# EdwardSmith1884/GEOMetrics

Hardware: AMD Instinct MI355X
Metric: meshes/sec (sample+Chamfer+tri_dist+0N-GCN fwd+bwd), 2562 verts/3000 pts (higher is better)
Workload: dtype f32; 1 GPU; BASELINE config 5 shard: 8 independent 2562-vert/5120-face meshes per GPU, full loss (face sampling 3000 pts + Chamfer NN vs 3000 GT pts + tri_distance 3000x5120 + point-to-surface) on top of a 3-layer 0N-GCN 963-192-192-192, fwd+bwd, single process (no collective), Adam step; meshes_per_gpu=8, global_batch=8, parallelism=dp1, launch=hipgraph, gemm_selection=tunableop file

## Files before the change

### geometrics_amd/build.py

```python
import glob
import os
import subprocess
import sys

HERE = os.path.dirname(os.path.abspath(__file__))
CSRC = os.path.join(HERE, "csrc")
INCLUDE = os.path.join(os.path.dirname(HERE), "include")
LIBDIR = os.path.join(HERE, "lib")
LIB = os.path.join(LIBDIR, "libgeom_hip.so")
STAMP = os.path.join(LIBDIR, "libgeom_hip.digest")
SHIM = os.path.join(LIBDIR, "geom_torch_shim.so")
SHIM_SRC = os.path.join(CSRC, "torch_shim.cpp")

HIPCC_FLAGS = ["--offload-arch=gfx950", "-O3", "-std=c++17", "-ffp-contract=off", "-fPIC",
               "-fno-gpu-rdc", "-fno-slp-vectorize", "-Wall", "-Wno-unused-function"]


EXTRA_FLAGS = {"dense_gemm.hip": ["-mllvm", "-amdgpu-mfma-vgpr-form=1"],
               "zn_stack.hip": ["-mllvm", "-amdgpu-mfma-vgpr-form=1"],
               "deform_block.hip": ["-mllvm", "-amdgpu-mfma-vgpr-form=1"],
               "encoder_stack.hip": ["-mllvm", "-amdgpu-mfma-vgpr-form=1"]}


def sources():
    return sorted(glob.glob(os.path.join(CSRC, "*.hip")))


def source_digest():
    import hashlib
    h = hashlib.sha256()
    for path in sorted(sources() + glob.glob(os.path.join(CSRC, "*.h")) + glob.glob(os.path.join(INCLUDE, "*.h"))):
        h.update(os.path.basename(path).encode())
        with open(path, "rb") as f:
            h.update(f.read())
    return h.hexdigest()


def _stale():
    if not os.path.exists(LIB):
        return True
    if built_digest() not in (None, source_digest()):
        return True
    t = os.path.getmtime(LIB)
    deps = sources() + glob.glob(os.path.join(CSRC, "*.h")) + glob.glob(os.path.join(INCLUDE, "*.h"))
    return any(os.path.getmtime(d) > t for d in deps)


def build_shim(force=False, verbose=False):
    if not force and os.path.exists(SHIM) and os.path.getmtime(SHIM) >= max(os.path.getmtime(SHIM_SRC), os.path.getmtime(LIB)):
        return SHIM
    import sysconfig
    import torch
    from torch.utils import cpp_extension as ce
    tlib = ce.library_paths()[0]
    cmd = ["g++", "-O2", "-std=c++17", "-fPIC", "-shared", "-w", "-D__HIP_PLATFORM_AMD__=1", "-DUSE_ROCM=1",
           "-DTORCH_EXTENSION_NAME=geom_torch_shim", "-D_GLIBCXX_USE_CXX11_ABI=%d" % int(torch._C._GLIBCXX_USE_CXX11_ABI),
           "-I", INCLUDE, "-I", sysconfig.get_paths()["include"], "-I", "/opt/rocm/include"]
    for inc in ce.include_paths():
        cmd += ["-I", inc]
    cmd += [SHIM_SRC, "-o", SHIM, "-L", LIBDIR, "-lgeom_hip", "-L", tlib, "-ltorch", "-ltorch_cpu", "-ltorch_hip", "-lc10",
            "-lc10_hip", "-ltorch_python", "-Wl,-rpath,$ORIGIN", "-Wl,-rpath," + tlib]
    if verbose:
        print(" ".join(cmd))
    subprocess.check_call(cmd)
    return SHIM


def build(force=False, verbose=False):
    lib = build_lib(force, verbose)
    build_shim(force, verbose)
    return lib


def build_lib(force=False, verbose=False):
    if not force and not _stale():
        return LIB
    hipcc = os.environ.get("HIPCC", "/opt/rocm/bin/hipcc")
    os.makedirs(LIBDIR, exist_ok=True)
    objs = []
    procs = []
    for src in sources():
        obj = os.path.join(LIBDIR, os.path.basename(src)[:-4] + ".o")
        objs.append(obj)
        cmd = [hipcc] + HIPCC_FLAGS + EXTRA_FLAGS.get(os.path.basename(src), []) + ["-I", INCLUDE, "-I", CSRC, "-c", src, "-o", obj]
        if verbose:
            print(" ".join(cmd))
        procs.append((src, subprocess.Popen(cmd, stdout=subprocess.PIPE, stderr=subprocess.STDOUT)))
    for src, p in procs:
        out, _ = p.communicate()
        if p.returncode != 0:
            raise RuntimeError("hipcc failed on %s:\n%s" % (src, out.decode(errors="replace")))
        if verbose and out:
            print(out.decode(errors="replace"))
    cmd = [hipcc, "--offload-arch=gfx950", "-shared", "-fPIC", "-fno-gpu-rdc"] + objs + ["-o", LIB]
    subprocess.check_call(cmd)
    with open(STAMP, "w") as f:
        f.write(source_digest() + "\n")
    return LIB


def built_digest():
    try:
        with open(STAMP) as f:
            return f.read().strip() or None
    except OSError:
        return None


if __name__ == "__main__":
    print(build(force="--force" in sys.argv, verbose=True))
```

### geometrics_amd/dense.py

```python
import ctypes

import torch

from . import _lib


def supported(cin, c, rows=1):
    return 0 < c <= 192 and c % 16 == 0 and cin > 0 and rows * max(cin, c) < 2 ** 30


def plan(rows, cin, c):
    ok = supported(cin, c, rows)
    pair = ok and cin <= 192 and cin % 4 == 0 and rows >= 512
    ok = ok and c % 48 == 0
    pair = pair and ok
    return {"fwd": "lib", "dx": "mfma" if pair else "lib", "dw": "mfma" if ok and rows >= 512 else "lib", "pair": pair}


def forward(x, w, out=None):
    rows, cin = x.shape
    c = w.shape[1]
    out = torch.empty(rows, c, dtype=torch.float32, device=x.device) if out is None else out
    with torch.cuda.device(x.device):
        _lib.call("geom_dense_fwd_f32", rows, cin, c, x.data_ptr(), w.data_ptr(), 0, None, out.data_ptr(), None, None)
    return out


def forward_split(x, w, bias, ksplit, out, sup, mask):
    rows, cin = x.shape
    c = w.shape[1]
    with torch.cuda.device(x.device):
        _lib.call("geom_dense_fwd_f32", rows, cin, c, x.data_ptr(), w.data_ptr(), ksplit, _lib.ptr(bias), out.data_ptr(),
                  sup.data_ptr(), _lib.ptr(mask))


def backward_input(g, w, out=None):
    rows, c = g.shape
    cin = w.shape[0]
    out = torch.empty(rows, cin, dtype=torch.float32, device=g.device) if out is None else out
    with torch.cuda.device(g.device):
        _lib.call("geom_dense_bwd_input_f32", rows, cin, c, g.data_ptr(), w.data_ptr(), out.data_ptr())
    return out


def weight_workspace(rows, cin, c, device):
    n = int(_lib.lib().geom_dense_bwd_weight_workspace_floats(rows, cin, c))
    return torch.empty(n, dtype=torch.float32, device=device)


launch_probe = None


def backward_weight_partials(x, g, workspace, want_colsum=False):
    rows, cin = x.shape
    c = g.shape[1]
    probe = launch_probe
    with torch.cuda.device(x.device):
        if probe is not None:
            start, end = torch.cuda.Event(enable_timing=True), torch.cuda.Event(enable_timing=True)
            start.record()
        _lib.call("geom_dense_bwd_weight_f32", rows, cin, c, x.data_ptr(), g.data_ptr(), workspace.data_ptr(),
                  1 if want_colsum else 0)
        if probe is not None:
            end.record()
            probe.append((rows, cin, c, start, end))


def backward_pair(x, g, w, grad_x, workspace, want_colsum=False):
    rows, cin = x.shape
    c = g.shape[1]
    with torch.cuda.device(x.device):
        _lib.call("geom_dense_bwd_f32", rows, cin, c, x.data_ptr(), g.data_ptr(), w.data_ptr(), grad_x.data_ptr(),
                  workspace.data_ptr(), 1 if want_colsum else 0)


def reduce(jobs, stream=None):
    n = len(jobs)
    if n == 0:
        return
    if n > _lib.DENSE_MAX_LAYERS:
        for i in range(0, n, _lib.DENSE_MAX_LAYERS):
            reduce(jobs[i:i + _lib.DENSE_MAX_LAYERS], stream)
        return
    ints = lambda k: (ctypes.c_int * n)(*[j[k] for j in jobs])
    ptrs = lambda k: (ctypes.c_void_p * n)(*[None if j[k] is None else j[k].data_ptr() for j in jobs])
    dev = jobs[0][3].device
    with torch.cuda.device(dev):
        _lib.check(_lib.status("geom_dense_reduce_f32", n, ints(0), ints(1), ints(2), ptrs(3), ptrs(4), ptrs(5), stream=stream),
                   "geom_dense_reduce_f32")


def backward_weight(x, g, want_bias=False):
    rows, cin = x.shape
    c = g.shape[1]
    ws = weight_workspace(rows, cin, c, x.device)
    backward_weight_partials(x, g, ws, want_bias)
    gw = torch.empty(cin, c, dtype=torch.float32, device=x.device)
    gb = torch.empty(c, dtype=torch.float32, device=x.device) if want_bias else None
    reduce([(rows, cin, c, ws, gw, gb)])
    return gw, gb


def any_supported(rows, cin, c):
    return rows >= 256 and cin > 0 and c > 0 and rows * max(cin, c) * 4 < 2 ** 31 - 1


def _row_major(t):
    return t.dim() == 2 and t.stride(1) == 1 and t.stride(0) >= t.shape[1]


def gemm(a, b, trans_a=False, trans_b=False, out=None, workspace=None):
    if not (_row_major(a) and _row_major(b)):
        raise ValueError("gemm operands must be 2-D with contiguous rows")
    for name, t in (("a", a), ("b", b), ("out", out), ("workspace", workspace)):
        if t is None:
            continue
        if not t.is_cuda or t.dtype != torch.float32:
            raise ValueError("gemm: %s must be a float32 tensor on a HIP device (got %s on %s)" % (name, t.dtype, t.device))
        if t.device != a.device:
            raise ValueError("gemm: %s is on %s, a on %s" % (name, t.device, a.device))
    k, m = (a.shape if trans_a else a.shape[::-1])
    n, kb = (b.shape if trans_b else b.shape[::-1])
    if k != kb:
        raise ValueError("gemm: summed extents differ (%d vs %d)" % (k, kb))
    if out is None:
        out = torch.empty(m, n, dtype=torch.float32, device=a.device)
    elif not _row_major(out) or tuple(out.shape) != (m, n):
        raise ValueError("gemm: out must be [%d, %d] with contiguous rows" % (m, n))
    need = int(_lib.lib().geom_gemm_workspace_floats(m, n, k))
    if need and (workspace is None or workspace.numel() < need):
        workspace = torch.empty(need, dtype=torch.float32, device=a.device)
    with torch.cuda.device(a.device):
        _lib.call("geom_gemm_f32", m, n, k, a.data_ptr(), a.stride(0), 1 if trans_a else 0, b.data_ptr(), b.stride(0),
                  0 if trans_b else 1, out.data_ptr(), out.stride(0), _lib.ptr(workspace) if need else None, need)
    return out


def split_bf16_planes(w):
    if not (w.is_cuda and w.dtype == torch.float32 and w.dim() == 2 and w.is_contiguous()):
        raise ValueError("split_bf16_planes: a contiguous 2-D float32 tensor on a HIP device")
    k, n = w.shape
    kpad = int(_lib.lib().geom_split_bf16_kpad(k))
    planes = torch.empty(3, n, kpad, dtype=torch.int16, device=w.device)
    with torch.cuda.device(w.device):
        _lib.call("geom_split_bf16_planes_f32", k, n, w.data_ptr(), planes.data_ptr())
    return planes


def gemm_split_bf16(a, planes, terms=6, out=None):
    if not (a.is_cuda and a.dtype == torch.float32 and a.dim() == 2 and a.is_contiguous()):
        raise ValueError("gemm_split_bf16: a contiguous 2-D float32 tensor on a HIP device")
    m, k = a.shape
    n = planes.shape[1]
    if planes.shape[2] != int(_lib.lib().geom_split_bf16_kpad(k)):
        raise ValueError("gemm_split_bf16: the planes belong to another k")
    out = torch.empty(m, n, dtype=torch.float32, device=a.device) if out is None else out
    with torch.cuda.device(a.device):
        _lib.call("geom_gemm_split_bf16_f32", m, k, n, a.data_ptr(), planes.data_ptr(), out.data_ptr(), int(terms))
    return out
```

### geometrics_amd/products.py

```python
import os
import threading
from collections import namedtuple

import torch

from . import backward_pass as _pass
from . import dense as _dense_kernels
from . import gemm_tuning


class _Slabs:
    def __init__(self, slots):
        self.open = {}
        self.slots = max(2, int(slots))

    def take(self, kind, shape, device, descending=False):
        shape = tuple(shape)
        key = (kind, shape, device, descending)
        slots = self.slots
        cur = self.open.get(key)
        if cur is None or cur[1] == slots:
            cur = self.open[key] = [torch.empty((slots,) + shape, dtype=torch.float32, device=device), 0]
        index = slots - 1 - cur[1] if descending else cur[1]
        cur[1] += 1
        return cur[0][index]


_active = threading.local()


def current_slabs():
    return getattr(_active, "slabs", None)


class weight_gradient_batching:

    def __init__(self, depth=4):
        self.depth = depth

    def __enter__(self):
        self.outer = current_slabs()
        _active.slabs = _Slabs(self.depth) if torch.is_grad_enabled() else None
        return self

    def __exit__(self, *exc):
        _active.slabs = self.outer
        return False


def _new_like(t, kind, arena, descending=False):
    if arena is None:
        return torch.empty_like(t)
    return arena.take(kind, t.shape, t.device, descending)


def _regular_run(tensors):
    first = tensors[0]
    if len(tensors) == 1:
        return first, 0
    base = first.untyped_storage().data_ptr()
    if any(t.untyped_storage().data_ptr() != base or t.stride() != first.stride() for t in tensors):
        return None
    step = tensors[1].storage_offset() - first.storage_offset()
    if step <= 0 or any(tensors[i + 1].storage_offset() - tensors[i].storage_offset() != step for i in range(len(tensors) - 1)):
        return None
    return first, step


def _launch_weight_products(jobs):
    i = 0
    while i < len(jobs):
        first = jobs[i]
        j = i + 1
        while (j < len(jobs) and jobs[j].x.shape == first.x.shape and jobs[j].g.shape == first.g.shape
               and jobs[j].stream == first.stream):
            j += 1
        group = jobs[i:j]
        with torch.cuda.stream(first.stream), torch.no_grad():
            runs = [_regular_run([getattr(job, name) for job in group]) for name in ("x", "g", "out")] if len(group) > 1 else None
            if runs and all(runs):
                xb, gb, ob = (torch.as_strided(run[0], (len(group),) + tuple(t.shape), (run[1],) + tuple(t.stride()))
                              for run, t in zip(runs, (first.x, first.g, first.out)))
                torch.bmm(xb.transpose(1, 2), gb, out=ob)
            else:
                for job in group:
                    dw = route(job.x.shape[0], job.x.shape[1], job.g.shape[1], True, True, True, True, False, use_any_shape_products).dw
                    _weight_product(dw, job.x, job.g, out=job.out)
        i = j


use_any_shape_products = True

own_dense_products = None


def _own_products_preferred():
    if own_dense_products is not None:
        return bool(own_dense_products)
    env = os.environ.get("GEOM_OWN_PRODUCTS")
    if env is not None:
        return env not in ("", "0")
    return gemm_tuning.status == "library default (tuning file rejected)"


Route = namedtuple("Route", "forward dx dw node")


def route(rows, cin, c, w_requires_grad, w_contiguous, x_contiguous, batched, own, any_allowed):
    plan = _dense_kernels.plan(rows, cin, c)
    split = plan["dw"] == "mfma"
    any_shape = any_allowed and not split and _dense_kernels.any_supported(rows, cin, c)
    lib_or_own = "own" if (own and w_contiguous and c % 16 == 0 and rows >= 512 and _dense_kernels.supported(cin, c, rows)) else "lib"
    forward = "any" if any_shape and w_contiguous else lib_or_own
    if batched:
        return Route(forward, lib_or_own, "any" if any_shape else "lib", True)
    if split and w_requires_grad:
        if x_contiguous and w_contiguous:
            return Route(forward, "pair" if plan["pair"] else lib_or_own, "split", True)
        return Route(forward, lib_or_own, "lib", lib_or_own == "own")
    if forward == "any":
        return Route("any", "any", "any", True)
    return Route(forward, lib_or_own, "lib", lib_or_own == "own")


def _input_gradient(kind, g, w2, out=None):
    if kind == "any":
        return _dense_kernels.gemm(g, w2, trans_b=True, out=out)
    if kind == "own":
        return _dense_kernels.backward_input(g, w2, out=out)
    return torch.matmul(g, w2.t()) if out is None else torch.mm(g, w2.t(), out=out)


def _weight_product(kind, x2, g2, out=None):
    if kind == "any" and x2.stride(1) == 1 and g2.stride(1) == 1 and (out is None or (out.dim() == 2 and out.stride(1) == 1)):
        return _dense_kernels.gemm(x2, g2, trans_a=True, out=out)
    return torch.mm(x2.t(), g2) if out is None else torch.mm(x2.t(), g2, out=out)


def product_gradients(x, g, w, w_ref, route, need_x, need_w, arena=None, dx=None, leaf=None):
    w2 = w.reshape(w.shape[-2:])
    cin, c = w2.shape
    x2, g2 = x.reshape(-1, cin), g.view(-1, c)
    rows = g2.shape[0]
    need_x = need_x and dx is None
    if route.dw == "split" and need_w:
        ws = _dense_kernels.weight_workspace(rows, cin, c, x.device)
        if need_x and route.dx == "pair":
            dx = torch.empty_like(x)
            _dense_kernels.backward_pair(x2, g2, w2, dx.view(rows, cin), ws)
        else:
            if need_x and leaf is not None and _pass.may_postpone_input_gradient(leaf):
                late = torch.empty(rows, cin, dtype=x.dtype, device=x.device)
                _pass.postpone_input_gradient(lambda: _input_gradient(route.dx, g2, w2, out=late), late, leaf)
            elif need_x:
                dx = _input_gradient(route.dx, g2, w2).view(x.shape)
            _dense_kernels.backward_weight_partials(x2, g2, ws)
        return dx, _pass.weight_gradient(w_ref, w, rows, cin, c, ws)
    if need_x:
        dx = _input_gradient(route.dx, g if arena is not None and route.dx == "lib" else g2, w2).view(x.shape)
    grad_w = None
    if need_w:
        param = w_ref() if arena is not None else None
        if param is not None and x2.is_contiguous() and _pass.may_defer(param, opted_in=True):
            grad_w = arena.take("dW", w.shape, w.device, descending=True)
            _pass.postpone_weight_product(x2, g2, grad_w, w_ref, _launch_weight_products)
        else:
            grad_w = _weight_product(route.dw, x2, g2).view(w.shape)
    return dx, grad_w


class _Product(torch.autograd.Function):

    @staticmethod
    def forward(ctx, x, w, route, arena):
        ctx.route, ctx.arena = route, arena
        ctx.w_ref = _pass.parameter_ref(w, ctx, ctx.needs_input_grad[1])
        x, out = _forward(route.forward, x, w.reshape(w.shape[-2:]))
        ctx.save_for_backward(x, w)
        return out

    @staticmethod
    def backward(ctx, grad):
        x, w = ctx.saved_tensors
        dx, dw = product_gradients(x, grad.contiguous(), w, ctx.w_ref, ctx.route, ctx.needs_input_grad[0], ctx.needs_input_grad[1],
                                   ctx.arena, leaf=x)
        return dx, dw, None, None


def _forward(kind, x, w2):
    if kind == "lib":
        return x, torch.matmul(x, w2)
    x2 = x.reshape(-1, x.shape[-1])
    if not x2.is_contiguous():
        x2 = x2.contiguous()
        x = x2.view(x.shape)
    out = _dense_kernels.gemm(x2, w2) if kind == "any" else _dense_kernels.forward(x2, w2)
    return x, out.view(x.shape[:-1] + (w2.shape[1],))


def _dense(x, w):
    if not (x.is_cuda and x.dtype == torch.float32 and w.dtype == torch.float32
            and (w.dim() == 2 or (w.dim() == 3 and w.shape[0] == 1)) and x.shape[-1] == w.shape[-2]):
        return torch.matmul(x, w.squeeze(0) if w.dim() == 3 else w)
    differentiable = torch.is_grad_enabled() and (x.requires_grad or w.requires_grad)
    arena = current_slabs() if differentiable else None
    cin = x.shape[-1]
    r = route(x.numel() // max(cin, 1), cin, w.shape[-1], w.requires_grad, w.is_contiguous(),
              x.is_contiguous() or x.reshape(-1, cin).is_contiguous(), arena is not None, _own_products_preferred(),
              use_any_shape_products)
    if differentiable and r.node:
        return _Product.apply(x, w, r, arena)
    return _forward(r.forward, x, w.reshape(w.shape[-2:]))[1]
```

### include/geom_hip.h

```cpp
#ifndef GEOM_HIP_H
#define GEOM_HIP_H

#include <stddef.h>
#include <stdint.h>

#ifdef __cplusplus
extern "C" {
#endif

#define GEOM_ABI_VERSION 16

#define GEOM_EINVAL   (-1)
#define GEOM_ETOOBIG  (-2)
#define GEOM_EUNSUPPORTED (-3)

#define GEOM_FLAG_REF_TAIL_TRUNC 1u
#define GEOM_FLAG_FIX_REGION6    2u
#define GEOM_FLAG_TRI_BRUTE_FORCE 4u
#define GEOM_FLAG_NN_FMA 8u

#define GEOM_FLAG_TRI_WS_READY 16u

int geom_abi_version(void);
const char *geom_strerror(int code);

int geom_chamfer_nn_f32(int b, int n, const float *xyz, int m, const float *xyz2,
                        float *result, int *result_i, float *result2, int *result2_i,
                        unsigned flags, void *stream);

int64_t geom_chamfer_nn_culled_workspace_floats(int b, int n, int m);
int geom_chamfer_nn_culled_f32(int b, int n, const float *xyz, int m, const float *xyz2, const int *order1, const int *order2,
                               float *result, int *result_i, float *result2, int *result2_i, unsigned flags, float *workspace,
                               void *stream);

int geom_tri_distance_f32(int b, int n, const float *xyz, int m,
                          const float *tri1, const float *tri2, const float *tri3,
                          float *dist, int *point, int *index, unsigned flags, void *stream);

int geom_tri_distance_indexed_f32(int b, int n, const float *xyz, int nv, const float *verts,
                                  int nf, const int64_t *faces,
                                  float *dist, int *point, int *index, unsigned flags, void *stream);

size_t geom_tri_distance_workspace_bytes(int b, int n, int m);
int geom_tri_distance_ws_f32(int b, int n, const float *xyz, int m,
                             const float *tri1, const float *tri2, const float *tri3, const int *order,
                             float *dist, int *point, int *index, unsigned flags,
                             void *workspace, size_t workspace_bytes, void *stream);
int geom_tri_distance_indexed_ws_f32(int b, int n, const float *xyz, int nv, const float *verts,
                                     int nf, const int64_t *faces, const int *order,
                                     float *dist, int *point, int *index, unsigned flags,
                                     void *workspace, size_t workspace_bytes, void *stream);

int geom_tri_surface_fwd_f32(int b, int n, const float *xyz, int nv, const float *verts, int nf,
                             const int64_t *faces, const int *order, float *dist, int *point, int *index,
                             float *sqdist, float *closest, float *weights, unsigned flags, void *workspace,
                             size_t workspace_bytes, void *stream);

int geom_face_areas_f32(int b, int nv, const float *verts, int nf, const int64_t *faces,
                        float *areas, void *stream);
int geom_draw_samples_f32(int b, int nv, const float *verts, int nf, const int64_t *faces, int num,
                          const float *uniforms, int64_t *choices, float *u, float *v, void *stream);
int geom_draw_samples_rng_f32(int b, int nv, const float *verts, int nf, const int64_t *faces, int num,
                              uint64_t *rng_state, int64_t *choices, float *u, float *v, float *points,
                              void *stream);
int geom_sample_faces_fwd_f32(int b, int nv, const float *verts, int nf, const int64_t *faces,
                              int num, const int64_t *choices, const float *u, const float *v,
                              float *points, void *stream);
int geom_sample_faces_bwd_f32(int b, int nv, int nf, const int64_t *faces,
                              int num, const int64_t *choices, const float *u, const float *v,
                              const float *grad_points, float *grad_verts, void *stream);

int geom_chamfer_grad_f32(int b, int n, const float *src, int m, const float *dst,
                          const int *idx, const float *coef_dev, float coef_host,
                          float *grad_src, int accumulate, float *grad_dst, void *stream);

int geom_p2tri_loss_fwd_f32(int b, int n, const float *xyz, int nv, const float *verts,
                            int nf, const int64_t *faces, const int *option, const int *index,
                            float *sqdist, float *closest, float *weights, void *stream);
int geom_p2tri_loss_bwd_f32(int b, int n, const float *xyz, int nv, int nf, const int64_t *faces,
                            const int *index, const float *closest, const float *weights,
                            const float *coef_dev, float coef_host, float *grad_verts, void *stream);

int geom_sum_f32(int64_t n, const float *x, float scale, float *out, void *stream);

int geom_sample_chamfer_bwd_f32(int b, int nv, int nf, const int64_t *faces, int num,
                                const int64_t *choices, const float *u, const float *v,
                                const float *points, int n_other, const float *other,
                                const int *idx, int via_nn, const float *coef_dev, float coef_host,
                                float *grad_verts, void *stream);
int geom_surface_loss_bwd_f32(int b, int nv, int nf, const int64_t *faces, int num, const int64_t *choices,
                              const float *u, const float *v, const float *points, int n_gt, const float *gt,
                              const int *idx_g, const int *index, const float *closest, const float *weights,
                              const float *coef_dev, float coef_sample, float coef_tri, float *grad_verts,
                              void *stream);

int geom_zn_gcn_aggregate_fwd_f32(int b, int nv, int c, int k, const int *rowptr, const int *col,
                                  const float *val, const float *support, const float *bias,
                                  int act, float *out, void *stream);
int64_t geom_zn_gcn_bwd_scratch_floats(int b, int nv, int c);
int64_t geom_zn_gcn_bwd_partial_rows(int b, int nv, int c, int k, int ell_w);
#define GEOM_COLSUM_MAX_JOBS 32
int geom_colsum_batch_f32(int count, const float *const *partials, const int *rows, const int *cols,
                          float *const *outs, void *stream);
int geom_zn_gcn_aggregate_bwd_f32(int b, int nv, int c, int k, const int *rowptrT, const int *colT,
                                  const float *valT, const float *grad_out, const float *out,
                                  int act, float *grad_support, float *grad_bias, float *scratch,
                                  void *stream);

int64_t geom_zn_gcn_relu_mask_words(int b, int nv, int c, int k);
int geom_zn_gcn_aggregate_ell_fwd_f32(int b, int nv, int c, int k, int w, const int *ell_col,
                                      const float *ell_val, const int *over_ptr, const int *over_col,
                                      const float *over_val, const float *support, const float *bias,
                                      int act, float *out, uint16_t *relu_mask, void *stream);
int geom_zn_gcn_aggregate_ell_bwd_f32(int b, int nv, int c, int k, int w, const int *ell_colT,
                                      const float *ell_valT, const int *over_ptrT, const int *over_colT,
                                      const float *over_valT, const float *grad_out, const float *out,
                                      const uint16_t *relu_mask, int act, float *grad_support,
                                      float *grad_bias, float *scratch, void *stream);

#define GEOM_DENSE_MAX_LAYERS 8
#define GEOM_DENSE_MAX_REDUCE_JOBS 32
int geom_dense_fwd_f32(int rows, int cin, int c, const float *x, const float *w, int ksplit, const float *bias,
                       float *out, float *sup, uint16_t *mask, void *stream);
int geom_dense_bwd_input_f32(int rows, int cin, int c, const float *g, const float *w, float *grad_x, void *stream);
int64_t geom_dense_bwd_weight_workspace_floats(int rows, int cin, int c);
int geom_dense_bwd_weight_f32(int rows, int cin, int c, const float *x, const float *g, float *workspace,
                              int want_colsum, void *stream);
int geom_dense_bwd_f32(int rows, int cin, int c, const float *x, const float *g, const float *w, float *grad_x,
                       float *workspace, int want_colsum, void *stream);
int geom_dense_reduce2_f32(int count, const int *rows, const int *cin, const int *c, const float *const *workspaces,
                           float *const *grad_w, float *const *grad_bias, int ncs, const float *const *cs_partials,
                           const int *cs_rows, const int *cs_cols, float *const *cs_outs, void *stream);
int geom_dense_reduce_adam_f32(int count, const int *rows, const int *cin, const int *c, const float *const *workspaces,
                               float *const *grad_w, float *const *w_p, float *const *w_m, float *const *w_v, int ncs,
                               const float *const *cs_partials, const int *cs_rows, const int *cs_cols, float *const *cs_outs,
                               float *const *b_p, float *const *b_m, float *const *b_v, float lr, float beta1, float beta2,
                               float eps, float *state, void *stream);
int geom_dense_reduce_f32(int count, const int *rows, const int *cin, const int *c, const float *const *workspaces,
                          float *const *grad_w, float *const *grad_bias, void *stream);

int geom_zn_gcn_aggregate_ell_head_fwd_f32(int b, int nv, int c, int k, int w, const int *ell_col,
                                           const float *ell_val, const int *over_ptr, const int *over_col,
                                           const float *over_val, const float *support, const float *bias,
                                           int act, float *out, uint16_t *relu_mask, const float *base,
                                           float scale, float *pos, void *stream);
int geom_zn_gcn_aggregate_ell_head_bwd_f32(int b, int nv, int c, int k, int w, const int *ell_colT,
                                           const float *ell_valT, const int *over_ptrT, const int *over_colT,
                                           const float *over_valT, const float *grad_pos, float scale,
                                           const uint16_t *relu_mask, int act, float *grad_support,
                                           float *grad_bias, float *scratch, void *stream);

int64_t geom_zn_layer_partial_rows(int b, int nv);
int geom_zn_layer_fwd_f32(int b, int nv, int c, int k, int ell_w, const int *ell_col, const float *ell_val,
                          const float *s_prev, const float *bias_prev, int act, const float *w, int n_out,
                          float *x_out, uint16_t *relu_mask, float *s_out, float *wt_out, void *stream);
int geom_zn_layer_bwd_f32(int b, int nv, int c, int k, int ell_w, const int *ell_col_t, const float *ell_val_t,
                          const float *grad_out, const float *out, const uint16_t *relu_mask, int act,
                          const float *grad_pos, float head_scale, const float *wt, int n_in, float *g_out,
                          float *grad_in, float *colsum_partial, void *stream);

typedef struct geom_deform_fwd {
    int b, nv, c, k, ell_w;
    const float *s_in, *bias;
    const int *ell_col; const float *ell_val;
    const int *tail_col; const float *tail_val;
    const float *bn_w, *bn_b;
    float *run_mean, *run_var;
    int training; float momentum, eps;
    int relu;
    const float *res; int res_ld; float scale;
    float *z_out, *x_out, *save_mean, *save_invstd;
    const float *w_next; float *s_out;
    const float *w_head; float *s_head;
    int vpx;
} geom_deform_fwd;
typedef struct geom_deform_bwd {
    int b, nv, c, k, ell_w;
    const float *dz_up;
    const int *ell_col_t; const float *ell_val_t;
    const int *tail_col_t; const float *tail_val_t;
    float *ds_up; const float *wt_up;
    const float *g, *g2;
    int g_ld, g2_ld;
    const float *z, *bn_w, *bn_b, *save_mean, *save_invstd;
    int relu, has_res; float scale;
    float *grad_res, *dz, *grad_bn_w, *grad_bn_b, *colsum;
    const float *ds_head, *w_head, *x_top; float *dw_head;
    int vpx;
} geom_deform_bwd;
#define GEOM_DEFORM_CHAIN_MAX 13
int geom_deform_chain_fits(int nv);
int geom_deform_chain_fwd_f32(int count, const geom_deform_fwd *layers, int *done, void *stream);
int geom_deform_chain_bwd_f32(int count, const geom_deform_bwd *layers, int *done, float *ds_first, void *stream);
int geom_deform_pack_weights_zero_f32(int count, const float *const *w, float *fwd, float *bwd, int *zero, int zero_words,
                                      void *stream);
typedef struct geom_deform_infer {
    int b, nv, c, k, ell_w;
    const float *s_in, *bias;
    const int *ell_col; const float *ell_val;
    const int *tail_col; const float *tail_val;
    const float *bn_w, *bn_b;
    const float *run_mean, *run_var;
    float eps;
    int relu;
    const float *res; int res_ld; float scale;
    float *x_out;
    const float *w_next; float *s_out;
    const float *w_head; float *s_head;
} geom_deform_infer;
int geom_deform_infer_fwd_f32(const geom_deform_infer *args, void *stream);
int geom_split_bf16_kpad(int k);
int geom_split_bf16_planes_f32(int k, int n, const float *w, uint16_t *planes, void *stream);
int geom_gemm_split_bf16_f32(int m, int k, int n, const float *a, const uint16_t *planes, float *c, int terms, void *stream);

int64_t geom_stage_regularisers_blocks(int b, int nv, int nf);
int geom_stage_regularisers_fwd_f32(int b, int nv, const float *prev, int prev_batched, const float *cur, int nf,
                                    const int64_t *faces, const int *rowptr, const int *col, const float *inv_deg,
                                    float c_lap, float c_move, float c_edge, float *lapd, float *partial, void *stream);
int geom_stage_regularisers_bwd_f32(int b, int nv, const float *prev, int prev_batched, const float *cur, int nf,
                                    const int64_t *faces, const int *rowptr, const int *col, const float *inv_deg,
                                    const int *vf_ptr, const int *vf_item, float c_lap, float c_move, float c_edge,
                                    const float *lapd, const float *gout, float *grad_prev, float *grad_cur, void *stream);

#define GEOM_SUM_MAX_TENSORS 8
int geom_sum_tensors_f32(int count, const float *const *tensors, int64_t n, float *out, void *stream);
int geom_sum_tensors_rows_f32(int count, const float *const *tensors, const int64_t *lds, int64_t rows, int width, float *out,
                              void *stream);

int geom_camera_info_f32(int b, const float *param, float *cam_mat, float *cam_pos, void *stream);

#define GEOM_DEFORM_MAX_PACK 16
#define GEOM_DEFORM_TAIL 32
int geom_deform_pack_weights_f32(int count, const float *const *w, float *fwd, float *bwd, void *stream);
int geom_deform_layer_fwd_f32(const geom_deform_fwd *args, void *stream);
int geom_deform_layer_bwd_f32(const geom_deform_bwd *args, void *stream);
#define GEOM_DEFORM_WIDE_MAX_B 64
int geom_deform_layer_wide_fwd_f32(const geom_deform_fwd *args, void *stream);
int geom_deform_layer_wide_bwd_f32(const geom_deform_bwd *args, void *stream);

int64_t geom_gemm_workspace_floats(int m, int n, int k);
int geom_gemm_f32(int m, int n, int k, const float *a, int64_t lda, int a_km, const float *b, int64_t ldb, int b_kn,
                  float *c, int64_t ldc, float *workspace, int64_t workspace_floats, void *stream);

int geom_vertex_head_fwd_f32(int64_t rows, int c, const float *base, const float *feat, float scale,
                             float *pos, void *stream);
int geom_vertex_head_bwd_f32(int64_t rows, int c, const float *grad_pos, float scale, float *grad_feat,
                             void *stream);

int geom_laplacian_f32(int b, int nv, const int *rowptr, const int *col, const float *inv_deg,
                       const float *x, int transpose, float *out, void *stream);
int geom_edge_sqlen_fwd_f32(int b, int nv, const float *verts, int nf, const int64_t *faces,
                            float *per_face, void *stream);
int geom_edge_sqlen_bwd_f32(int b, int nv, const float *verts, int nf, const int64_t *faces,
                            const float *coef_dev, float coef_host, float *grad_verts, void *stream);

int geom_vertex_bn_fwd_f32(int b, int nv, int c, const float *x, const float *weight, const float *bias,
                           float *running_mean, float *running_var, int training, float momentum, float eps,
                           int relu, const float *residual, int residual_ld, float scale,
                           float *out, float *save_mean, float *save_invstd, void *stream);
int geom_vertex_bn_bwd_f32(int b, int nv, int c, const float *x, const float *grad_out, const float *weight,
                           const float *bias, const float *save_mean, const float *save_invstd, int relu,
                           int has_residual, float scale, float *grad_x, float *grad_residual,
                           float *grad_weight, float *grad_bias, const float *grad_out2, void *stream);

size_t geom_pool_features_bwd_workspace_bytes(int b, int nv, int levels, const int *dims);
#define GEOM_POOL_MAX_LEVELS 8
int geom_pool_features_fwd_ld_f32(int b, int nv, const float *verts, const float *cam_mat, const float *cam_pos, int levels,
                                  const float *const *blocks, const int *channels, const int *dims, float *out, int64_t out_ld,
                                  void *stream);
int geom_pool_features_fwd_fronts_f32(int b, int nv, const float *verts, const float *cam_mat, const float *cam_pos, int levels,
                                      const float *const *blocks, const int *channels, const int *dims, float *out,
                                      int64_t out_ld, int n_fronts, const float *const *fronts, const int *widths,
                                      const int *cols, float *buf, void *stream);
int geom_pool_features_bwd_ld_f32(int b, int nv, const float *verts, const float *cam_mat, const float *cam_pos, int levels,
                                  const float *const *blocks, const int *channels, const int *dims, const float *grad_out,
                                  int64_t grad_ld, float *const *grad_blocks, float *grad_verts, void *workspace,
                                  size_t workspace_bytes, void *stream);

typedef struct geom_surface_cull {
    const int *gt_order;
    const float *gt_index;
    float *sample_index;
    const int *faces_in_order;
} geom_surface_cull;
int64_t geom_nn_cull_index_floats(int b, int n);
int geom_nn_cull_index_f32(int b, int n, const float *xyz, const int *order, float *index, void *stream);

int geom_surface_prepare_f32(int b, int nv, const float *verts, int nf, const int64_t *faces, int num,
                             uint64_t *rng_state, int64_t *choices, float *u, float *v, float *points, int n_gt,
                             const int *tri_order, unsigned flags, void *workspace, size_t workspace_bytes,
                             int *prepared, const geom_surface_cull *cull, void *stream);

size_t geom_surface_tail_counters_offset(int b, int n_gt, int nf);
typedef struct geom_surface_tail {
    const int64_t *choices;
    float scale_sample, scale_other;
    int want_order;
    float *loss;
    int finalized;
} geom_surface_tail;
int geom_surface_scan_f32(int b, int n_gt, const float *gt, int num, const float *points, float *sq_gt, int *idx_p,
                          float *sq_pred, int *idx_g, int nv, const float *verts, int nf, const int64_t *faces,
                          const int *tri_order, float *tri_dist, int *option, int *index, float *sq, float *closest,
                          float *weights, const float *u, const float *v, float coef_sample, float coef_other,
                          int *order_scratch, unsigned flags, void *workspace, size_t workspace_bytes,
                          int *records_written, const geom_surface_cull *cull, geom_surface_tail *tail, void *stream);

int64_t geom_surface_order_words(int b, int nf, int num, int n_gt);
int geom_surface_finalize_f32(int b, int nf, int num, const int64_t *choices, const float *u, const float *v,
                              const float *points, int n_gt, const float *gt, const int *idx_g, const int *idx_p,
                              const int *index, const float *closest, const float *weights, const float *sq_sample,
                              const float *sq_other, float scale_sample, float scale_other, float coef_sample,
                              float coef_other, int want_order, int records_ready, int *order, float *loss,
                              void *stream);
int geom_surface_gather_f32(int b, int nv, int nf, const int *vf_ptr, const int *vf_item, int num, int n_gt,
                            int has_other, const int *order, const float *grad, float *grad_verts, void *stream);
int geom_surface_finalize_w_f32(int b, int nf, int num, const int64_t *choices, const float *u, const float *v,
                                const float *points, int n_gt, const float *gt, const int *idx_g, const int *idx_p,
                                const int *index, const float *closest, const float *weights, const float *sq_sample,
                                const float *sq_other, float scale_sample, float scale_other, float coef_sample,
                                float coef_other, int want_order, int records_ready, int *order, float *loss,
                                const float *mesh_weight, void *stream);
int geom_surface_gather_w_f32(int b, int nv, int nf, const int *vf_ptr, const int *vf_item, int num, int n_gt,
                              int has_other, const int *order, const float *grad, const float *mesh_weight,
                              float *grad_verts, void *stream);

int64_t geom_segment_max_workspace_bytes(int nseg, int c, int64_t max_len);
int geom_segment_max_fwd_f32(int nseg, const int64_t *offsets, int64_t max_len, int c, const float *x,
                             float *out, int *arg, void *workspace, int64_t workspace_bytes, void *stream);
int geom_segment_max_bwd_f32(int nseg, const int64_t *offsets, int64_t total_rows, int c,
                             const float *grad_out, const int *arg, float *grad_x, void *stream);

int geom_encoder_layer_fwd_f32(int b, int nv, int c, int k, int n, const int *rowptr, const int *col, const float *val,
                               const float *s, int64_t lds, const float *bias, int act, const float *w, int64_t ldw,
                               float *out, int64_t ldo, float *x_out, int64_t ldx, void *stream);
int geom_encoder_layer_bwd_f32(int b, int nv, int c, int k, int n, const int *rowptrT, const int *colT, const float *valT,
                               const float *g, int64_t ldg, const float *x_saved, int64_t ldx, int act, const float *w,
                               int64_t ldw, float *out, int64_t ldo, float *t_out, int64_t ldt, void *stream);
int geom_latent_l1_fwd_f32(int b, int l, const float *pred, const float *target, const float *on, float weight, float *loss,
                           void *stream);
int geom_latent_l1_bwd_f32(int b, int l, const float *pred, const float *target, const float *on, float weight,
                           const float *grad_loss, float *grad_pred, void *stream);

#define GEOM_ADAM_MAX_TENSORS 64
#define GEOM_ADAM_STATE_WORDS 2112
int geom_adam_step_f32(int count, float *const *params, const float *const *grads, float *const *exp_avg,
                       float *const *exp_avg_sq, const int64_t *sizes, float lr, float beta1, float beta2,
                       float eps, float grad_scale, float *state, int advance, void *stream);
int64_t geom_adam_table_bytes(int count, int64_t total_blocks);
int geom_adam_table_step_f32(int count, const void *table, int64_t total_blocks, const float *lr, float beta1, float beta2,
                             float eps, float grad_scale, float *state, int advance, void *stream);

#ifdef __cplusplus
}
#endif
#endif
```

Baseline: 17780 meshes/s.

## Add split-bf16 MFMA kernel for wide-input dense backward dx

Adds a HIP kernel that computes the input gradient of a dense layer with 192 outputs and wide input. It splits fp32 operands into three bf16 planes and accumulates six bf16 MFMA products so the result stays near fp32 accuracy. The products fallback routes large wide-input dx products (at least 16384 rows) to this kernel instead of torch.matmul. It also adds a per-call weight plane-conversion launch and rounding behaviour that differs from the fp32 GEMM.

After: 18620 meshes/s, median of 6. +4.7%, better.

```diff
diff --git a/geometrics_amd/build.py b/geometrics_amd/build.py
--- a/geometrics_amd/build.py
+++ b/geometrics_amd/build.py
@@ -19,7 +19,8 @@
 EXTRA_FLAGS = {"dense_gemm.hip": ["-mllvm", "-amdgpu-mfma-vgpr-form=1"],
                "zn_stack.hip": ["-mllvm", "-amdgpu-mfma-vgpr-form=1"],
                "deform_block.hip": ["-mllvm", "-amdgpu-mfma-vgpr-form=1"],
-               "encoder_stack.hip": ["-mllvm", "-amdgpu-mfma-vgpr-form=1"]}
+               "encoder_stack.hip": ["-mllvm", "-amdgpu-mfma-vgpr-form=1"],
+               "dense_dx_split_bf16.hip": ["-mllvm", "-amdgpu-mfma-vgpr-form=1"]}
 
 
 def sources():
diff --git a/geometrics_amd/csrc/dense_dx_split_bf16.hip b/geometrics_amd/csrc/dense_dx_split_bf16.hip
--- /dev/null
+++ b/geometrics_amd/csrc/dense_dx_split_bf16.hip
@@ -0,0 +1,296 @@
+#include "geom_common.h"
+#include <type_traits>
+
+namespace {
+
+typedef float f32x4 __attribute__((ext_vector_type(4)));
+typedef __bf16 bf16x8 __attribute__((ext_vector_type(8)));
+typedef unsigned u32x4 __attribute__((ext_vector_type(4)));
+
+constexpr int DX_THREADS = 256;
+constexpr int DX_K = 192;
+constexpr int DX_KB = DX_K / 32;
+constexpr int DX_NT = 2;
+constexpr int DX_MAX_RB = 6;
+constexpr int DX_ROW_BYTES = DX_K * 2;
+constexpr int DX_PLANE = DX_MAX_RB * 16 * DX_ROW_BYTES;
+constexpr int DX_LDS = 3 * DX_PLANE;
+
+__device__ __forceinline__ unsigned bf16_bits_of(float x) { return (unsigned)__builtin_bit_cast(unsigned short, (__bf16)x); }
+__device__ __forceinline__ float bf16_value_of(unsigned bits) { return __uint_as_float(bits << 16); }
+__device__ __forceinline__ void split3(float a, unsigned &b0, unsigned &b1, unsigned &b2)
+{
+    b0 = bf16_bits_of(a);
+    const float r1 = a - bf16_value_of(b0);
+    b1 = bf16_bits_of(r1);
+    const float r2 = r1 - bf16_value_of(b1);
+    b2 = bf16_bits_of(r2);
+}
+
+__host__ __device__ __forceinline__ size_t dx_frag_index(int group, int kb, int t, int plane, int lane)
+{
+    return ((((size_t)group * DX_KB + kb) * DX_NT + t) * 3 + plane) * 64 + lane;
+}
+
+__global__ __launch_bounds__(256) void dx_planes_kernel(int cin, int cinpad, const float *w, uint4 *planes)
+{
+    const int i = blockIdx.x * 256 + threadIdx.x;
+    if (i >= cinpad * (DX_K / 8)) return;
+    const int col = i / (DX_K / 8), k8 = i - col * (DX_K / 8);
+    unsigned e[8][3];
+#pragma unroll
+    for (int j = 0; j < 8; ++j) e[j][0] = e[j][1] = e[j][2] = 0;
+    if (col < cin) {
+        const float4 lo = *reinterpret_cast<const float4 *>(w + (size_t)col * DX_K + 8 * k8);
+        const float4 hi = *reinterpret_cast<const float4 *>(w + (size_t)col * DX_K + 8 * k8 + 4);
+        const float v[8] = {lo.x, lo.y, lo.z, lo.w, hi.x, hi.y, hi.z, hi.w};
+#pragma unroll
+        for (int j = 0; j < 8; ++j) split3(v[j], e[j][0], e[j][1], e[j][2]);
+    }
+    const int tile = col >> 4;
+#pragma unroll
+    for (int pl = 0; pl < 3; ++pl)
+        planes[dx_frag_index(tile / DX_NT, k8 >> 2, tile % DX_NT, pl, 16 * (k8 & 3) + (col & 15))] =
+            make_uint4(e[0][pl] | (e[1][pl] << 16), e[2][pl] | (e[3][pl] << 16), e[4][pl] | (e[5][pl] << 16), e[6][pl] | (e[7][pl] << 16));
+}
+
+constexpr unsigned DX_NOWHERE = 0x80000000u;
+__device__ __forceinline__ __amdgpu_buffer_rsrc_t dx_rsrc(const void *ptr, int64_t bytes)
+{
+    return __builtin_amdgcn_make_buffer_rsrc(const_cast<void *>(ptr), 0, (int)bytes, 0x00020000);
+}
+
+struct DxArgs {
+    const float *g;
+    const void *wp;
+    float *dx;
+    int rows, cin, cinpad, ldx, spread;
+};
+
+__device__ __forceinline__ int lds_chunk(int r, int q) { return r * DX_ROW_BYTES + ((q ^ ((r >> 1) & 7)) << 4); }
+
+__device__ __forceinline__ void dx_terms(const bf16x8 (&a)[3], const bf16x8 (&b)[DX_NT][3], f32x4 (&hi)[DX_NT], f32x4 (&lo)[DX_NT])
+{
+#pragma unroll
+    for (int t = 0; t < DX_NT; ++t) hi[t] = __builtin_amdgcn_mfma_f32_16x16x32_bf16(a[0], b[t][0], hi[t], 0, 0, 0);
+#pragma unroll
+    for (int t = 0; t < DX_NT; ++t) lo[t] = __builtin_amdgcn_mfma_f32_16x16x32_bf16(a[0], b[t][1], lo[t], 0, 0, 0);
+#pragma unroll
+    for (int t = 0; t < DX_NT; ++t) lo[t] = __builtin_amdgcn_mfma_f32_16x16x32_bf16(a[1], b[t][0], lo[t], 0, 0, 0);
+#pragma unroll
+    for (int t = 0; t < DX_NT; ++t) lo[t] = __builtin_amdgcn_mfma_f32_16x16x32_bf16(a[1], b[t][1], lo[t], 0, 0, 0);
+#pragma unroll
+    for (int t = 0; t < DX_NT; ++t) lo[t] = __builtin_amdgcn_mfma_f32_16x16x32_bf16(a[0], b[t][2], lo[t], 0, 0, 0);
+#pragma unroll
+    for (int t = 0; t < DX_NT; ++t) lo[t] = __builtin_amdgcn_mfma_f32_16x16x32_bf16(a[2], b[t][0], lo[t], 0, 0, 0);
+}
+
+__device__ __forceinline__ void dx_store(const DxArgs &p, __amdgpu_buffer_rsrc_t r_dx, int rb, int grp, int lane, const f32x4 (&hi)[DX_NT],
+                                         const f32x4 (&lo)[DX_NT])
+{
+    const int row = rb * 16 + 4 * (lane >> 4), col = grp * (16 * DX_NT) + (lane & 15);
+#pragma unroll
+    for (int e = 0; e < 4; ++e)
+#pragma unroll
+        for (int t = 0; t < DX_NT; ++t) {
+            const unsigned off = row + e < p.rows && col + 16 * t < p.cin ? (unsigned)(((row + e) * p.ldx + col + 16 * t) * 4) : DX_NOWHERE;
+#ifdef DX_PROBE_NO_STORE
+            if (p.ldx < 0)
+#endif
+            __builtin_amdgcn_raw_buffer_store_b32(__float_as_uint(hi[t][e] + lo[t][e]), r_dx, off, 0, 0);
+        }
+}
+
+template <int N>
+__device__ __forceinline__ void dx_sweep(const DxArgs &p, const unsigned char *lds, int wave, int lane, int rb0)
+{
+    const int lr = lane & 15, lg = lane >> 4;
+    const int ngroups = p.cinpad / (16 * DX_NT);
+    bf16x8 bf[2][DX_KB][DX_NT][3];
+    bf16x8 af[2][3];
+    const __amdgpu_buffer_rsrc_t r_w = dx_rsrc(p.wp, (int64_t)3 * p.cinpad * DX_K * 2);
+    const __amdgpu_buffer_rsrc_t r_dx = dx_rsrc(p.dx, ((int64_t)(p.rows - 1) * p.ldx + p.cin) * 4);
+    auto a_frags = [&](int set, int rbi, int kb) {
+#pragma unroll
+        for (int pl = 0; pl < 3; ++pl)
+            af[set][pl] = *reinterpret_cast<const bf16x8 *>(lds + pl * DX_PLANE + lds_chunk(rbi * 16 + lr, 4 * kb + lg));
+    };
+    auto b_frags = [&](int set, int grp, int kb) {
+        const unsigned base = grp < ngroups ? (unsigned)(dx_frag_index(grp, 0, 0, 0, lane) * 16) : DX_NOWHERE;
+#pragma unroll
+        for (int t = 0; t < DX_NT; ++t)
+#pragma unroll
+            for (int pl = 0; pl < 3; ++pl)
+                bf[set][kb][t][pl] = __builtin_bit_cast(bf16x8, __builtin_amdgcn_raw_buffer_load_b128(r_w, base + (unsigned)(dx_frag_index(0, kb, t, pl, 0) * 16), 0, 0));
+    };
+    auto group = [&](auto set_c, int grp, int next) {
+        constexpr int S = decltype(set_c)::value;
+#pragma unroll
+        for (int rbi = 0; rbi < N; ++rbi) {
+            f32x4 hi[DX_NT], lo[DX_NT];
+#pragma unroll
+            for (int t = 0; t < DX_NT; ++t) hi[t] = lo[t] = (f32x4){0.f, 0.f, 0.f, 0.f};
+#ifndef DX_PROBE_NO_REFILL
+#pragma unroll
+            for (int kb = rbi * DX_KB / N; kb < (rbi + 1) * DX_KB / N; ++kb) b_frags(S ^ 1, next, kb);
+#endif
+#pragma unroll
+            for (int kb = 0; kb < DX_KB; ++kb) {
+                const int s = kb & 1;
+#ifndef DX_PROBE_NO_LDS
+                if (kb + 1 < DX_KB) a_frags(s ^ 1, rbi, kb + 1);
+                else a_frags(0, rbi + 1 < N ? rbi + 1 : 0, 0);
+                __builtin_amdgcn_sched_barrier(0);
+#endif
+                dx_terms(af[s], bf[S][kb], hi, lo);
+            }
+            dx_store(p, r_dx, rb0 + rbi, grp, lane, hi, lo);
+        }
+    };
+
+    if (wave >= ngroups) return;
+#pragma unroll
+    for (int kb = 0; kb < DX_KB; ++kb) b_frags(0, wave, kb);
+#ifdef DX_PROBE_NO_REFILL
+#pragma unroll
+    for (int kb = 0; kb < DX_KB; ++kb) b_frags(1, wave, kb);
+#endif
+    a_frags(0, 0, 0);
+    for (int grp = wave; grp < ngroups; grp += 8) {
+        group(std::integral_constant<int, 0>(), grp, grp + 4);
+        if (grp + 4 < ngroups) group(std::integral_constant<int, 1>(), grp + 4, grp + 8);
+    }
+}
+
+__device__ __forceinline__ void dx_stray(const DxArgs &p, const unsigned char *lds, int lane, int lds_rb, int rb, int grp)
+{
+    const int lr = lane & 15, lg = lane >> 4;
+    const __amdgpu_buffer_rsrc_t r_w = dx_rsrc(p.wp, (int64_t)3 * p.cinpad * DX_K * 2);
+    const __amdgpu_buffer_rsrc_t r_dx = dx_rsrc(p.dx, ((int64_t)(p.rows - 1) * p.ldx + p.cin) * 4);
+    bf16x8 b[DX_KB][DX_NT][3];
+#pragma unroll
+    for (int kb = 0; kb < DX_KB; ++kb)
+#pragma unroll
+        for (int t = 0; t < DX_NT; ++t)
+#pragma unroll
+            for (int pl = 0; pl < 3; ++pl)
+                b[kb][t][pl] = __builtin_bit_cast(bf16x8, __builtin_amdgcn_raw_buffer_load_b128(r_w, (unsigned)(dx_frag_index(grp, kb, t, pl, lane) * 16), 0, 0));
+    f32x4 hi[DX_NT], lo[DX_NT];
+#pragma unroll
+    for (int t = 0; t < DX_NT; ++t) hi[t] = lo[t] = (f32x4){0.f, 0.f, 0.f, 0.f};
+#pragma unroll
+    for (int kb = 0; kb < DX_KB; ++kb) {
+        bf16x8 a[3];
+#pragma unroll
+        for (int pl = 0; pl < 3; ++pl) a[pl] = *reinterpret_cast<const bf16x8 *>(lds + pl * DX_PLANE + lds_chunk(lds_rb * 16 + lr, 4 * kb + lg));
+        dx_terms(a, b[kb], hi, lo);
+    }
+    dx_store(p, r_dx, rb, grp, lane, hi, lo);
+}
+
+__global__ __launch_bounds__(DX_THREADS, 1) void dx_split_kernel(DxArgs p)
+{
+    extern __shared__ __attribute__((aligned(16))) unsigned char lds[];
+    const int tid = threadIdx.x, wave = tid >> 6, lane = tid & 63;
+    const int nrb = (p.rows + 15) >> 4;
+    int rb0 = (int)((int64_t)blockIdx.x * nrb / gridDim.x), n = (int)((int64_t)(blockIdx.x + 1) * nrb / gridDim.x) - rb0;
+    int stray_rb = -1, stray_grp = 0;
+    if (p.spread) {
+        const int ngroups = p.cinpad / (16 * DX_NT), share = nrb / (int)gridDim.x;
+        rb0 = blockIdx.x * share, n = share;
+        if ((int)blockIdx.x < (nrb - share * (int)gridDim.x) * ngroups) stray_rb = share * gridDim.x + blockIdx.x / ngroups, stray_grp = blockIdx.x % ngroups;
+    }
+
+#ifndef DX_PROBE_NO_PROLOGUE
+    {
+        const __amdgpu_buffer_rsrc_t r_g = dx_rsrc(p.g, (int64_t)p.rows * DX_K * 4);
+        u32x4 v[3 * DX_MAX_RB];
+#pragma unroll
+        for (int i = 0; i < 3 * DX_MAX_RB; ++i) {
+            const int q = tid + DX_THREADS * i, r = q / (DX_K / 4);
+            const int row = r < 16 * n ? rb0 * 16 + r : stray_rb * 16 + r - 16 * n;
+            const unsigned off = r < 16 * n || (stray_rb >= 0 && r < 16 * n + 16) ? (unsigned)((row * DX_K + 4 * (q - r * (DX_K / 4))) * 4) : DX_NOWHERE;
+            v[i] = __builtin_amdgcn_raw_buffer_load_b128(r_g, off, 0, 0);
+        }
+#pragma unroll
+        for (int i = 0; i < 3 * DX_MAX_RB; ++i) {
+            const int q = tid + DX_THREADS * i, r = q / (DX_K / 4), c4 = q - r * (DX_K / 4);
+            unsigned e[4][3];
+            split3(__uint_as_float(v[i].x), e[0][0], e[0][1], e[0][2]);
+            split3(__uint_as_float(v[i].y), e[1][0], e[1][1], e[1][2]);
+            split3(__uint_as_float(v[i].z), e[2][0], e[2][1], e[2][2]);
+            split3(__uint_as_float(v[i].w), e[3][0], e[3][1], e[3][2]);
+            unsigned char *dst = lds + lds_chunk(r, c4 >> 1) + 8 * (c4 & 1);
+#pragma unroll
+            for (int pl = 0; pl < 3; ++pl)
+                *reinterpret_cast<uint2 *>(dst + pl * DX_PLANE) = make_uint2(e[0][pl] | (e[1][pl] << 16), e[2][pl] | (e[3][pl] << 16));
+        }
+    }
+#endif
+    __syncthreads();
+    switch (n) {
+    case 1: dx_sweep<1>(p, lds, wave, lane, rb0); break;
+    case 2: dx_sweep<2>(p, lds, wave, lane, rb0); break;
+    case 3: dx_sweep<3>(p, lds, wave, lane, rb0); break;
+    case 4: dx_sweep<4>(p, lds, wave, lane, rb0); break;
+    case 5: dx_sweep<5>(p, lds, wave, lane, rb0); break;
+    case 6: dx_sweep<6>(p, lds, wave, lane, rb0); break;
+    default: break;
+    }
+    if (stray_rb >= 0 && wave == 3) dx_stray(p, lds, lane, n, stray_rb, stray_grp);
+}
+
+int compute_units()
+{
+    static int cus[64];
+    int dev = 0;
+    if (hipGetDevice(&dev) != hipSuccess || dev < 0 || dev >= 64) return 256;
+    if (!cus[dev]) {
+        int n = 0;
+        cus[dev] = (hipDeviceGetAttribute(&n, hipDeviceAttributeMultiprocessorCount, dev) == hipSuccess && n > 0) ? n : 256;
+    }
+    return cus[dev];
+}
+
+}
+
+extern "C" int geom_dense_dx_split_cinpad(int cin) { return cin <= 0 ? 0 : (cin + 16 * DX_NT - 1) / (16 * DX_NT) * (16 * DX_NT); }
+
+extern "C" int geom_dense_dx_split_planes_f32(int cin, int c, const float *w, uint16_t *planes, void *stream)
+{
+    if (cin <= 0 || c <= 0) return GEOM_EINVAL;
+    if (c != DX_K) return GEOM_EUNSUPPORTED;
+    if (!w || !planes || ((uintptr_t)w & 15) || ((uintptr_t)planes & 15)) return GEOM_EINVAL;
+    const int cinpad = geom_dense_dx_split_cinpad(cin);
+    if ((int64_t)cinpad * DX_K * 6 >= (1LL << 31)) return GEOM_ETOOBIG;
+    const int frags = cinpad * (DX_K / 8);
+    hipLaunchKernelGGL(dx_planes_kernel, dim3((unsigned)((frags + 255) / 256)), dim3(256), 0, static_cast<hipStream_t>(stream), cin, cinpad, w,
+                       reinterpret_cast<uint4 *>(planes));
+    return geom::launch_status();
+}
+
+extern "C" int geom_dense_dx_split_f32(int rows, int cin, int c, const float *g, const uint16_t *planes, float *dx, int ldx, void *stream)
+{
+    if (rows < 0 || cin <= 0 || c <= 0 || ldx < cin) return GEOM_EINVAL;
+    if (c != DX_K) return GEOM_EUNSUPPORTED;
+    if (rows == 0) return 0;
+    if (!g || !planes || !dx || ((uintptr_t)g & 15) || ((uintptr_t)planes & 15) || ((uintptr_t)dx & 3)) return GEOM_EINVAL;
+    const int cinpad = geom_dense_dx_split_cinpad(cin);
+    if ((int64_t)cinpad * DX_K * 6 >= (1LL << 31) || (int64_t)rows * ldx * 4 >= (1LL << 31) || (int64_t)rows * DX_K * 4 >= (1LL << 31)) return GEOM_ETOOBIG;
+    DxArgs p{g, planes, dx, rows, cin, cinpad, ldx, 0};
+    static bool configured[64];
+    int dev = 0;
+    if (hipGetDevice(&dev) == hipSuccess && dev >= 0 && dev < 64 && !configured[dev]) {
+        if (hipFuncSetAttribute(reinterpret_cast<const void *>(dx_split_kernel), hipFuncAttributeMaxDynamicSharedMemorySize, DX_LDS) != hipSuccess)
+            return GEOM_EINVAL;
+        configured[dev] = true;
+    }
+    const int64_t nrb = ((int64_t)rows + 15) >> 4;
+    const int64_t cus = compute_units();
+    const int64_t rounds = (nrb + DX_MAX_RB * cus - 1) / (DX_MAX_RB * cus);
+    const int64_t grid = nrb < rounds * cus ? nrb : rounds * cus;
+    const int64_t left = nrb % grid;
+    p.spread = left > 0 && left * (cinpad / (16 * DX_NT)) <= grid;
+    hipLaunchKernelGGL(dx_split_kernel, dim3((unsigned)grid), dim3(DX_THREADS), DX_LDS, static_cast<hipStream_t>(stream), p);
+    return geom::launch_status();
+}
diff --git a/geometrics_amd/dense.py b/geometrics_amd/dense.py
--- a/geometrics_amd/dense.py
+++ b/geometrics_amd/dense.py
@@ -1,4 +1,5 @@
 import ctypes
+import os
 
 import torch
 
@@ -15,6 +16,63 @@
     ok = ok and c % 48 == 0
     pair = pair and ok
     return {"fwd": "lib", "dx": "mfma" if pair else "lib", "dw": "mfma" if ok and rows >= 512 else "lib", "pair": pair}
+
+
+WIDE_DX_MIN_ROWS = 16384
+
+
+def wide_dx_plan(rows, cin, c):
+    return c == 192 and cin > 192 and rows >= WIDE_DX_MIN_ROWS
+
+
+wide_dx = None
+
+
+def wide_dx_takes(g, w, out=None):
+    mode = wide_dx if wide_dx is not None else (os.environ.get("GEOM_WIDE_DX") or None)
+    if mode not in (None, "lib", "split"):
+        raise ValueError("GEOM_WIDE_DX / dense.wide_dx must be 'lib' or 'split' (got %r)" % (mode,))
+    if mode == "lib" or w.dim() != 2 or g.dim() < 2:
+        return False
+    cin, c = w.shape
+    rows = g.numel() // max(c, 1)
+    if not (c == 192 and g.shape[-1] == c and cin > 192 and rows >= 1 and rows * max(cin, c) < 2 ** 29):
+        return False
+    for t in (g, w) + (() if out is None else (out,)):
+        if not (t.is_cuda and t.dtype == torch.float32 and t.is_contiguous() and t.device == g.device):
+            return False
+    if g.data_ptr() % 16 or w.data_ptr() % 16 or (out is not None and tuple(out.shape) != (rows, cin)):
+        return False
+    return mode == "split" or wide_dx_plan(rows, cin, c)
+
+
+def wide_dx_planes(w):
+    if not (w.is_cuda and w.dtype == torch.float32 and w.dim() == 2 and w.is_contiguous()):
+        raise ValueError("wide_dx_planes: a contiguous 2-D float32 tensor on a HIP device")
+    cin, c = w.shape
+    planes = torch.empty(3 * int(_lib.lib().geom_dense_dx_split_cinpad(cin)) * c, dtype=torch.int16, device=w.device)
+    with torch.cuda.device(w.device):
+        _lib.call("geom_dense_dx_split_planes_f32", cin, c, w.data_ptr(), planes.data_ptr())
+    return planes
+
+
+def wide_dx_planes_matrix(planes):
+    nt = int(_lib.lib().geom_dense_dx_split_cinpad(1)) // 16
+    return planes.view(-1, 6, nt, 3, 4, 16, 8).permute(3, 0, 2, 5, 1, 4, 6).reshape(3, -1, 192)
+
+
+def backward_input_split(g, w, out=None):
+    rows, c = g.shape
+    cin = w.shape[0]
+    if not (g.is_cuda and g.dtype == torch.float32 and g.dim() == 2 and g.is_contiguous()):
+        raise ValueError("backward_input_split: g must be a contiguous float32 tensor on a HIP device")
+    planes = wide_dx_planes(w)
+    out = torch.empty(rows, cin, dtype=torch.float32, device=g.device) if out is None else out
+    if not (_row_major(out) and out.dtype == torch.float32 and out.device == g.device and tuple(out.shape) == (rows, cin)):
+        raise ValueError("backward_input_split: out must be a float32 [%d, %d] tensor with contiguous rows on g's device" % (rows, cin))
+    with torch.cuda.device(g.device):
+        _lib.call("geom_dense_dx_split_f32", rows, cin, c, g.data_ptr(), planes.data_ptr(), out.data_ptr(), out.stride(0) if rows > 1 else cin)
+    return out
 
 
 def forward(x, w, out=None):
diff --git a/geometrics_amd/products.py b/geometrics_amd/products.py
--- a/geometrics_amd/products.py
+++ b/geometrics_amd/products.py
@@ -128,6 +128,9 @@
         return _dense_kernels.gemm(g, w2, trans_b=True, out=out)
     if kind == "own":
         return _dense_kernels.backward_input(g, w2, out=out)
+    if _dense_kernels.wide_dx_takes(g, w2, out):
+        dx = _dense_kernels.backward_input_split(g.view(-1, g.shape[-1]), w2, out=out)
+        return dx if out is not None else dx.view(g.shape[:-1] + (w2.shape[0],))
     return torch.matmul(g, w2.t()) if out is None else torch.mm(g, w2.t(), out=out)
 
 
diff --git a/include/geom_hip.h b/include/geom_hip.h
--- a/include/geom_hip.h
+++ b/include/geom_hip.h
@@ -212,6 +212,9 @@
 int geom_split_bf16_kpad(int k);
 int geom_split_bf16_planes_f32(int k, int n, const float *w, uint16_t *planes, void *stream);
 int geom_gemm_split_bf16_f32(int m, int k, int n, const float *a, const uint16_t *planes, float *c, int terms, void *stream);
+int geom_dense_dx_split_cinpad(int cin);
+int geom_dense_dx_split_planes_f32(int cin, int c, const float *w, uint16_t *planes, void *stream);
+int geom_dense_dx_split_f32(int rows, int cin, int c, const float *g, const uint16_t *planes, float *dx, int ldx, void *stream);
 
 int64_t geom_stage_regularisers_blocks(int b, int nv, int nf);
 int geom_stage_regularisers_fwd_f32(int b, int nv, const float *prev, int prev_batched, const float *cur, int nf,
```
